# Vegeta2020/SE-SSD

Measured on NVIDIA H100. Metric: frames_per_sec, higher is better.
Workload: dtype f32

## Files before the change

### se-ssd_b200/csrc/bevconv_p2.cuh

```cuda
#pragma once
#include <cuda_fp16.h>

#include "tc_common.cuh"

namespace sessd {

constexpr int kP2TileU = 8, kP2TileV = 16;
constexpr int kP2MaxCopies = 6, kP2MaxRowsV = 18;
constexpr int kP2BStages = 6, kP2MaxBStages = 12;
constexpr int kP2MmaWarps = 8;
constexpr int kP2PatchWarp = 8, kP2WeightWarp = 9;
constexpr int kP2Threads = 320;
constexpr int kP2ThreadsRegA = 384, kP2RegsConsumer = 232, kP2RegsProducer = 40;
static_assert(2 * (kP2RegsConsumer - 168) <= 168 - kP2RegsProducer, "the consumers take what the producers release");
constexpr int kP2MaxSmem = 227 * 1024;
constexpr int kP2Chunk = 32;
constexpr int kP2ItemsHeader = 32;
enum { kP2Planes = 0, kP2SplitF16 = 1 };
enum { kP2NoProbe = 0, kP2ProbeClocks = 1, kP2ProbeLoads = 2 };

struct P2Params {
    int batch, cin, cout;
    int in_stride;
    int out_h, out_w;
// ... 27 lines not shown
    kProfItems,
    kProfSteps,
    kProfItemClk,
    kProfBFull,
    kProfPatchFull,
    kProfMmaWait,
    kProfEpilogue,
    kProfPatchEmpty,
    kProfPatchTotal,
    kProfBEmpty,
    kProfBTotal,
    kP2ProfWords = 16
};

__device__ __forceinline__ int p2_item_count(const P2Params &p) { return p.items ? __ldg(p.items) : p.total; }
__device__ __forceinline__ int p2_item(const P2Params &p, int k) { return p.items ? __ldg(p.items + kP2ItemsHeader + k) : k; }

struct P2ItemIndex { int rank, nb, t; };
__host__ __device__ __forceinline__ P2ItemIndex p2_item_index(int g, int nblocks, int tiles) {
    const int rank = g / (nblocks * tiles), rem = g - rank * (nblocks * tiles), nb = rem / tiles;
    return {rank, nb, rem - nb * tiles};
}

struct P2Item { int cls, n0, b, u0, v0, ntaps; };

__device__ __forceinline__ P2Item p2_decode(const P2Params &p, int g) {
    P2Item it;
    const P2ItemIndex ix = p2_item_index(g, p.nblocks, p.tiles);
    int t = ix.t;
    it.cls = p.cls_order[ix.rank];
    it.n0 = ix.nb * p.n_tile;
    const int tu = t % p.tiles_u; t /= p.tiles_u;
    const int tv = t % p.tiles_v;
    it.b = t / p.tiles_v;
    it.u0 = tu * kP2TileU; it.v0 = tv * kP2TileV;
    it.ntaps = p.cls_ntaps[it.cls];
    return it;
}

template <int N>
__device__ __forceinline__ void p2_wgmma(float *d, uint64_t da, uint64_t db, uint32_t accumulate) {
    if constexpr (N == 32) wgmma_f16_n32(d, da, db, accumulate);
    else if constexpr (N == 64) wgmma_f16_n64(d, da, db, accumulate);
    else if constexpr (N == 128) wgmma_f16_n128(d, da, db, accumulate);
    else wgmma_f16_n256(d, da, db, accumulate);
}

template <int N>
__device__ __forceinline__ void p2_wgmma_ra(float *d, const uint32_t *a, uint64_t db, uint32_t accumulate) {
    if constexpr (N == 32) wgmma_f16_ra_n32(d, a, db, accumulate);
    else if constexpr (N == 64) wgmma_f16_ra_n64(d, a, db, accumulate);
    else if constexpr (N == 128) wgmma_f16_ra_n128(d, a, db, accumulate);
    else wgmma_f16_ra_n256(d, a, db, accumulate);
}

__device__ __forceinline__ void p2_quad_transpose(const float *s, int q, float v[8]) {
    const bool odd = q & 1, up = q & 2;
    float a[2][2][2];
#pragma unroll
    for (int k = 0; k < 2; ++k)
#pragma unroll
        for (int e = 0; e < 2; ++e) {
            const float even_g = s[4 * (2 * k) + e], odd_g = s[4 * (2 * k + 1) + e];
            const float keep = odd ? odd_g : even_g;
            const float recv = __shfl_xor_sync(0xFFFFFFFFu, odd ? even_g : odd_g, 1);
            a[k][0][e] = odd ? recv : keep;
            a[k][1][e] = odd ? keep : recv;
        }
#pragma unroll
    for (int b = 0; b < 2; ++b)
#pragma unroll
        for (int e = 0; e < 2; ++e) {
            const float keep = up ? a[1][b][e] : a[0][b][e];
            const float recv = __shfl_xor_sync(0xFFFFFFFFu, up ? a[0][b][e] : a[1][b][e], 2);
            v[2 * b + e] = up ? recv : keep;
            v[2 * (2 + b) + e] = up ? keep : recv;
        }
}

template <bool PROFILE>
__device__ __forceinline__ long long p2_tick() {
    if constexpr (PROFILE) return clock64();
    return 0;
}
template <bool PROFILE>
__device__ __forceinline__ void p2_tock(long long &clk, long long t0) {
    if constexpr (PROFILE) clk += clock64() - t0;
}

__device__ __forceinline__ void p2_split_patch(const P2Params &p, const unsigned char *staging, unsigned char *planes, float s_in, int ctid) {
    const int rows = p.rows_v * kP2TileU;
    const int copy_in = p.staging_bytes / p.ncopies;
    const int items = p.ncopies * rows * 4;
    for (int i = ctid; i < items; i += kP2MmaWarps * 32) {
        const int j = i & 3, r = (i >> 2) % rows, c = (i >> 2) / rows;
        unsigned char *hi = planes + 2 * c * p.copy_bytes + r * 64 + ((j ^ ((r >> 1) & 3)) << 4);
        const float4 *src = reinterpret_cast<const float4 *>(staging + c * copy_in + r * 128 + j * 32);
        const float4 a = src[0], b = src[1];
        const float x[8] = {a.x * s_in, a.y * s_in, a.z * s_in, a.w * s_in, b.x * s_in, b.y * s_in, b.z * s_in, b.w * s_in};
        __align__(16) __half h[8], l[8];
#pragma unroll
        for (int t = 0; t < 8; ++t) { h[t] = __float2half_rn(x[t]); l[t] = __float2half_rn(x[t] - __half2float(h[t])); }
        *reinterpret_cast<uint4 *>(hi) = *reinterpret_cast<const uint4 *>(h);
        *reinterpret_cast<uint4 *>(hi + p.copy_bytes) = *reinterpret_cast<const uint4 *>(l);
    }
    asm volatile("fence.proxy.async.shared::cta;\n" ::: "memory");
    asm volatile("bar.sync 1, %0;\n" ::"n"(kP2MmaWarps * 32) : "memory");
}

template <int NT, int MODE, bool REGA = false, int PROBE = kP2NoProbe>
__global__ void __launch_bounds__(REGA ? kP2ThreadsRegA : kP2Threads, 1) bev_conv_p2_kernel(const __grid_constant__ CUtensorMap map_a,
                                                                   const __grid_constant__ CUtensorMap map_b,
                                                                   const float *__restrict__ scale, const float *__restrict__ shift,
                                                                   const float *__restrict__ resid, float *__restrict__ out_f32,
                                                                   __half *__restrict__ out_planes, P2Params p) {
    static_assert(!REGA || MODE == kP2Planes, "register-fed A reads the TMA-written planes");
    constexpr bool PROFILE = PROBE != kP2NoProbe, LOADS_ONLY = PROBE == kP2ProbeLoads;
    extern __shared__ unsigned char smem_raw[];
    unsigned char *tiles = (unsigned char *)(((uintptr_t)smem_raw + 1023) & ~(uintptr_t)1023);
    unsigned char *patches = tiles + p.bring_bytes;
    unsigned char *staging = patches + p.npatch * p.patch_bytes;
    uint64_t *bars = (uint64_t *)(staging + p.npatch * p.staging_bytes);
    uint64_t *patch_full = bars, *patch_empty = bars + 2, *b_full = bars + 4, *b_empty = bars + 4 + kP2MaxBStages;
    uint32_t *s_aoff = (uint32_t *)(b_empty + kP2MaxBStages);
    float *s_scale = (float *)(((uintptr_t)(s_aoff + 4 * 9) + 15) & ~(uintptr_t)15), *s_shift = s_scale + p.cout;

    const int warp = threadIdx.x >> 5, lane = threadIdx.x & 31;
    if (threadIdx.x == kP2PatchWarp * 32) prefetch_tensormap(&map_a);
    if (threadIdx.x == kP2WeightWarp * 32) prefetch_tensormap(&map_b);
    const int nchunks = p.cin / kP2Chunk;
// ... 197 lines not shown
                        first = false;
                        if constexpr (PROFILE) ++clk[kProfSteps];
                        { const long long t0 = p2_tick<PROFILE>(); wgmma_wait<1>(); p2_tock<PROFILE>(clk[kProfMmaWait], t0); }
                        if (lane == 0) {
                            if (prevS >= 0) mbar_arrive(&b_empty[prevS]);
                            if (prev_pb >= 0) mbar_arrive(&patch_empty[prev_pb]);
                        }
                        prevS = S;
                        prev_pb = (tap == ntaps - 1) ? pb : -1;
                        if (++S == p.bstages) { S = 0; bph ^= 1u; }
                    }
                    if (p.npatch == 1) {
                        { const long long t0 = p2_tick<PROFILE>(); wgmma_wait<0>(); p2_tock<PROFILE>(clk[kProfMmaWait], t0); }
                        if (lane == 0) {
                            mbar_arrive(&b_empty[prevS]);
                            mbar_arrive(&patch_empty[pb]);
                        }
                        prevS = prev_pb = -1;
                    }
                    if (++pb == p.npatch) { pb = 0; pph ^= 1u; }
                }
            }
            { const long long t0 = p2_tick<PROFILE>(); wgmma_wait<0>(); p2_tock<PROFILE>(clk[kProfMmaWait], t0); }
            const long long t_epi = p2_tick<PROFILE>();
            wgmma_fence_regs<NT>(acc);
            if (lane == 0) {
                if (prevS >= 0) mbar_arrive(&b_empty[prevS]);
                if (prev_pb >= 0) mbar_arrive(&patch_empty[prev_pb]);
            }
#pragma unroll
            for (int i = 0; i < kAcc; ++i) acc[i] = acc[kAcc + i] + acc[i];
            const P2Item it = p2_decode(p, g);
            const int q = lane & 3;
            const int r0 = wg * 64 + wq * 16 + (lane >> 2);
            bool rows_ok[2];
            size_t opixs[2];
#pragma unroll
            for (int h = 0; h < 2; ++h) {
                const int r = r0 + 8 * h;
                const int lv = r / kP2TileU, lu = r % kP2TileU;
                const int gu = it.u0 + lu, gv = it.v0 + lv;
                rows_ok[h] = it.b < p.batch && gu < p.grid_u && gv < p.grid_v;
                const int ou = gu * p.out_stride + p.cls_off_u[it.cls], ov = gv * p.out_stride + p.cls_off_v[it.cls];
                const int oy = p.u_is_x ? ov : ou, ox = p.u_is_x ? ou : ov;
                opixs[h] = ((size_t)it.b * p.out_h + (size_t)oy) * p.out_w + (size_t)ox;
            }
#pragma unroll
            for (int j = 0; j < (LOADS_ONLY ? 0 : NT / 32); ++j)
#pragma unroll
                for (int h = 0; h < 2; ++h) {
                    const bool row_ok = rows_ok[h];
                    const size_t opix = opixs[h];
                    float v[8], o[8] = {};
                    p2_quad_transpose(acc + 16 * j + 2 * h, q, v);
                    const int n = it.n0 + 32 * j + 8 * q;
                    const size_t off = opix * p.cout + n;
                    if (row_ok && n < p.cout) {
                        float sc[8], sh[8];
#pragma unroll
                        for (int t = 0; t < 8; t += 4) {
                            const float4 a = *reinterpret_cast<const float4 *>(s_scale + n + t);
                            const float4 b = *reinterpret_cast<const float4 *>(s_shift + n + t);
                            sc[t] = a.x; sc[t + 1] = a.y; sc[t + 2] = a.z; sc[t + 3] = a.w;
                            sh[t] = b.x; sh[t + 1] = b.y; sh[t + 2] = b.z; sh[t + 3] = b.w;
                        }
#pragma unroll
                        for (int t = 0; t < 8; ++t) {
                            o[t] = fmaf(v[t] * inv_sa, sc[t], sh[t]);
                            if (p.relu) o[t] = fmaxf(o[t], 0.f);
                        }
                        if (resid) {
#pragma unroll
                            for (int t = 0; t < 8; t += 4) {
                                const float4 rr = __ldg(reinterpret_cast<const float4 *>(resid + off + t));
                                o[t] += rr.x; o[t + 1] += rr.y; o[t + 2] += rr.z; o[t + 3] += rr.w;
                            }
                        }
#pragma unroll
                        for (int t = 0; t < 8; ++t) vmax = fmaxf(vmax, fabsf(o[t]));
                        if (out_planes) {
                            __align__(16) __half2 hi[4], lo[4];
#pragma unroll
                            for (int t = 0; t < 4; ++t) {
                                const float x0 = o[2 * t] * s_out, x1 = o[2 * t + 1] * s_out;
                                hi[t] = __floats2half2_rn(x0, x1);
                                const float2 f = __half22float2(hi[t]);
                                lo[t] = __floats2half2_rn(x0 - f.x, x1 - f.y);
                            }
                            *reinterpret_cast<uint4 *>(out_planes + off) = *reinterpret_cast<const uint4 *>(hi);
                            *reinterpret_cast<uint4 *>(out_planes + p.out_plane_stride + off) = *reinterpret_cast<const uint4 *>(lo);
                        }
                    }
                    if (out_f32) {
                        const bool up = q & 2;
                        float keep[4], recv[4];
#pragma unroll
                        for (int t = 0; t < 4; ++t) {
                            keep[t] = up ? o[4 + t] : o[t];
                            recv[t] = __shfl_xor_sync(0xFFFFFFFFu, up ? o[t] : o[4 + t], 2);
                        }
                        const int n_lo = it.n0 + 32 * j + 8 * (q & 1), c_lo = n_lo + 4 * (q >> 1);
                        const float4 w_lo = up ? make_float4(recv[0], recv[1], recv[2], recv[3]) : make_float4(keep[0], keep[1], keep[2], keep[3]);
                        const float4 w_hi = up ? make_float4(keep[0], keep[1], keep[2], keep[3]) : make_float4(recv[0], recv[1], recv[2], recv[3]);
                        if (row_ok && n_lo < p.cout) *reinterpret_cast<float4 *>(out_f32 + opix * p.cout + c_lo) = w_lo;
                        if (row_ok && n_lo + 16 < p.cout) *reinterpret_cast<float4 *>(out_f32 + opix * p.cout + c_lo + 16) = w_hi;
                    }
                }
// ... 274 lines not shown
```

### se-ssd_b200/csrc/spconv_cg.cu

```cuda
#include <cuda_fp16.h>

#include "tc_common.cuh"
#include "tile_lists.cuh"

namespace sessd {

constexpr int kCgBM = 128;
constexpr int kCgMaxK = 27;
constexpr int kCgProdWarps = 8;
constexpr int kCgMmaWarps = 8;
constexpr int kCgWeightWarp = kCgProdWarps + kCgMmaWarps;
constexpr int kCgThreads = (kCgWeightWarp + 1) * 32;

template <int CP, int COUT, int DEEP = 0>
struct CgCfg {
    static constexpr bool kWide = (CP == 64);
    static constexpr int kATile = (kWide ? 2 : 1) * kCgBM * 128;
    static constexpr int kBTile = (kWide ? 2 : 1) * COUT * 128;
    static constexpr int kStage = kATile + (kBTile + 1023) / 1024 * 1024;
    static constexpr int kStages = (kWide ? 2 : 4) * (DEEP ? 2 : 1);
    static constexpr int kMeta = kCgBM * kCgMaxK * 4  + kCgMaxK * 16  + 32 * 4  + 33 * 4  + 32 * 4  +
                                 3 * kStages * 8  + 24;
    static constexpr int kSmem = kStages * kStage + kMeta + 1024;
    static constexpr int kCPO = COUT > 32 ? 64 : 32;
};

struct CgArgs {
    const __half *planes;
    const float *in_info;
    const unsigned int *tiles;
    int tile_stride;
    const int *d_n_out;
    int kvol, max_out, relu;
    const float *scale, *shift;
    float gain, shift_max;
    float *out_f32;
    __half *out_planes;
    float *out_info;
};

__device__ __forceinline__ void cg_cp_async16(uint32_t smem_dst, const void *gsrc) {
    asm volatile("cp.async.cg.shared.global [%0], [%1], 16;\n" ::"r"(smem_dst), "l"(gsrc) : "memory");
}
__device__ __forceinline__ void cg_fence_proxy_async() { asm volatile("fence.proxy.async.shared::cta;\n" ::: "memory"); }
__device__ __forceinline__ void cg_sts_zero16(uint32_t saddr) {
    asm volatile("st.shared.v4.b32 [%0], {%1, %1, %1, %1};\n" ::"r"(saddr), "r"(0) : "memory");
}

template <int COUT>
__device__ __forceinline__ void cg_wgmma(float *d, uint64_t da, uint64_t db, uint32_t accumulate) {
    if constexpr (COUT == 32) wgmma_f16_n32(d, da, db, accumulate);
    else wgmma_f16_n64(d, da, db, accumulate);
}

template <int CP, int COUT, int DEEP>
__global__ void __launch_bounds__(kCgThreads, 1) spconv_cg_kernel(const __grid_constant__ CUtensorMap map_w, const CgArgs a) {
    using C = CgCfg<CP, COUT, DEEP>;
    const int n_out = min(*a.d_n_out, a.max_out);
    const int ntiles = (n_out + kCgBM - 1) / kCgBM;
    if ((int)blockIdx.x >= ntiles) return;
    const int kvol = a.kvol;
    if (threadIdx.x == kCgWeightWarp * 32) prefetch_tensormap(&map_w);

    extern __shared__ unsigned char smem_raw[];
    unsigned char *tiles = (unsigned char *)(((uintptr_t)smem_raw + 1023) & ~(uintptr_t)1023);
    uint32_t *s_list = (uint32_t *)(tiles + C::kStages * C::kStage);
    uint32_t *s_valid = s_list + kCgBM * kCgMaxK;
    int *s_cnt = (int *)(s_valid + kCgMaxK * 4);
    int *s_klist = s_cnt + 32;
    int *s_nact = s_klist + 32;
    int *s_off = s_nact + 1;
    uint64_t *bars = (uint64_t *)(((uintptr_t)(s_off + 32) + 7) & ~(uintptr_t)7);
    uint64_t *full_a = bars, *full_b = bars + C::kStages, *empty = bars + 2 * C::kStages;

    const int tid = threadIdx.x, warp = tid >> 5, lane = tid & 31;
    const uint32_t tiles_u32 = smem_u32(tiles);

    if (tid == 0) {
        for (int s = 0; s < C::kStages; ++s) { mbar_init(&full_a[s], kCgProdWarps / C::kStages); mbar_init(&full_b[s], 1); mbar_init(&empty[s], kCgMmaWarps); }
        asm volatile("fence.mbarrier_init.release.cluster;\n" ::: "memory");
    }
    for (int s = 0; s < C::kStages; ++s)
        for (int o = tid * 16; o < C::kATile; o += kCgThreads * 16) cg_sts_zero16(tiles_u32 + (uint32_t)(s * C::kStage + o));
    cg_fence_proxy_async();
    __syncthreads();

    const float amax_in = __ldg(a.in_info), s_in = __ldg(a.in_info + 1);
    const float inv_act = 1.f / s_in;
    const float s_out = pow2_scale_for_bound(amax_in * a.gain + a.shift_max);
    if (blockIdx.x == 0 && tid == 0 && a.out_info) a.out_info[1] = s_out;
    float vmax = 0.f;
    uint32_t dirty[4] = {0u, 0u, 0u, 0u};
    int st0 = 0;
    uint32_t ph0 = 0;

    for (int tile = blockIdx.x; tile < ntiles; tile += gridDim.x) {
        const int row0 = tile * kCgBM;
        const int rows = min(kCgBM, n_out - row0);
        {
            const unsigned int *rec = a.tiles + (size_t)tile * (size_t)a.tile_stride;
            const int c = (int)__ldg(rec + lane);
            unsigned int spec[4];
#pragma unroll
            for (int u = 0; u < 4; ++u) spec[u] = (tid + u * kCgThreads < kTlRows * kvol) ? __ldg(rec + kTlHeader + tid + u * kCgThreads) : 0u;
            const int incl = warp_incl_scan(c, lane);
            const int total = __shfl_sync(0xffffffffu, incl, 31);
            if (warp == 0) {
                s_cnt[lane] = c;
                s_off[lane] = incl - c;
                const unsigned int m = __ballot_sync(0xffffffffu, c > 0);
                if (c > 0) s_klist[__popc(m & ((1u << lane) - 1u))] = lane;
                if (lane == 0) *s_nact = __popc(m);
            }
            if (tid < kvol * 4) s_valid[tid] = __ldg(rec + kTlMask + tid);
#pragma unroll
            for (int u = 0; u < 4; ++u)
                if (tid + u * kCgThreads < total) s_list[tid + u * kCgThreads] = spec[u];
            for (int e = tid + 4 * kCgThreads; e < total; e += kCgThreads) s_list[e] = __ldg(rec + kTlHeader + e);
        }
        __syncthreads();
        const int nact = *s_nact;

        if (warp == kCgWeightWarp) {
            int s = st0;
            uint32_t ph = ph0;
            for (int j = 0; j < nact; ++j) {
                const int k = s_klist[j];
                mbar_wait(&empty[s], ph ^ 1u);
                if (elect_one()) {
                    mbar_expect_tx(&full_b[s], C::kBTile);
                    unsigned char *b_tile = tiles + s * C::kStage + C::kATile;
                    tma_load_4d(b_tile, &map_w, &full_b[s], 0, 0, 0, k);
                    tma_load_4d(b_tile + C::kBTile / 2, &map_w, &full_b[s], 0, 0, 1, k);
                }
                __syncwarp();
                if (++s == C::kStages) { s = 0; ph ^= 1u; }
            }
        } else if (warp >= kCgProdWarps) {
            const int cw = warp - kCgProdWarps, wg = cw >> 2, wq = cw & 3;
            constexpr int kAcc = COUT / 2;
            float acc_m[kAcc], acc_c[kAcc];
#pragma unroll
            for (int i = 0; i < kAcc; ++i) { acc_m[i] = 0.f; acc_c[i] = 0.f; }
            const uint32_t a_rows = (uint32_t)(wg * 64 * 128);
            int s = st0, prev = -1;
            uint32_t ph = ph0;
            for (int j = 0; j < nact; ++j) {
                mbar_wait(&full_b[s], ph);
                mbar_wait(&full_a[s], ph);
                const uint32_t st = tiles_u32 + (uint32_t)(s * C::kStage);
                const uint64_t dA = kDescSw128Hi | desc_lo(st + a_rows);
                const uint32_t first = j != 0 ? 1u : 0u;
                wgmma_fence();
                if constexpr (C::kWide) {
                    const uint64_t dAl = dA + ((kCgBM * 128) >> 4);
                    const uint64_t dBh = kDescSw128Hi | desc_lo(st + C::kATile);
                    const uint64_t dBl = dBh + ((COUT * 128) >> 4);
#pragma unroll
                    for (int kk = 0; kk < 4; ++kk) cg_wgmma<COUT>(acc_m, dA + 2 * kk, dBh + 2 * kk, first | (kk != 0));
#pragma unroll
                    for (int kk = 0; kk < 4; ++kk) cg_wgmma<COUT>(acc_c, dA + 2 * kk, dBl + 2 * kk, first | (kk != 0));
#pragma unroll
                    for (int kk = 0; kk < 4; ++kk) cg_wgmma<COUT>(acc_c, dAl + 2 * kk, dBh + 2 * kk, 1u);
                } else {
                    const uint64_t dBh = kDescSw64Hi | desc_lo(st + C::kATile);
                    const uint64_t dBl = dBh + ((COUT * 64) >> 4);
#pragma unroll
                    for (int kk = 0; kk < 2; ++kk) cg_wgmma<COUT>(acc_m, dA + 2 * kk, dBh + 2 * kk, first | (kk != 0));
#pragma unroll
                    for (int kk = 0; kk < 2; ++kk) cg_wgmma<COUT>(acc_c, dA + 2 * kk, dBl + 2 * kk, first | (kk != 0));
#pragma unroll
                    for (int kk = 0; kk < 2; ++kk) cg_wgmma<COUT>(acc_c, dA + 4 + 2 * kk, dBh + 2 * kk, 1u);
                }
                wgmma_commit();
                wgmma_wait<1>();
                if (prev >= 0 && lane == 0) mbar_arrive(&empty[prev]);
                prev = s;
                if (++s == C::kStages) { s = 0; ph ^= 1u; }
            }
            wgmma_wait<0>();
            wgmma_fence_regs<kAcc>(acc_m);
            wgmma_fence_regs<kAcc>(acc_c);
            if (prev >= 0 && lane == 0) mbar_arrive(&empty[prev]);
            const int r0 = wg * 64 + wq * 16 + (lane >> 2);
            const int c2 = 2 * (lane & 3);
#pragma unroll
            for (int h = 0; h < 2; ++h) {
                const int r = r0 + 8 * h;
                if (r >= rows) continue;
                const size_t orow = (size_t)(row0 + r);
#pragma unroll
                for (int g = 0; g < COUT / 8; ++g) {
                    const int n = 8 * g + c2, i = 4 * g + 2 * h;
                    const float2 sc = __ldg(reinterpret_cast<const float2 *>(a.scale + n));
                    const float2 sh = a.shift ? __ldg(reinterpret_cast<const float2 *>(a.shift + n)) : make_float2(0.f, 0.f);
                    float o0 = fmaf((acc_m[i] + acc_c[i]) * inv_act, sc.x, sh.x);
                    float o1 = fmaf((acc_m[i + 1] + acc_c[i + 1]) * inv_act, sc.y, sh.y);
                    if (a.relu) { o0 = fmaxf(o0, 0.f); o1 = fmaxf(o1, 0.f); }
                    vmax = fmaxf(vmax, fmaxf(fabsf(o0), fabsf(o1)));
                    if (a.out_f32) *reinterpret_cast<float2 *>(a.out_f32 + orow * COUT + n) = make_float2(o0, o1);
                    if (a.out_planes) {
                        const float x0 = o0 * s_out, x1 = o1 * s_out;
                        const __half2 hi = __floats2half2_rn(x0, x1);
                        const float2 f = __half22float2(hi);
                        const __half2 lo = __floats2half2_rn(x0 - f.x, x1 - f.y);
                        __half2 *dst = reinterpret_cast<__half2 *>(a.out_planes + orow * (2 * C::kCPO) + n);
                        dst[0] = hi;
                        dst[C::kCPO / 2] = lo;
                    }
                }
            }
        } else {
            constexpr int kGroupWarps = kCgProdWarps / C::kStages;
            constexpr int kGroupThreads = kGroupWarps * 32;
            constexpr int kOwnRows = kCgBM / kGroupWarps;
            constexpr int kOwnWords = kOwnRows / 32;
            constexpr int kLanesPerRow = C::kWide ? 16 : 8;
            constexpr int kRowsPerPass = kGroupThreads / kLanesPerRow;
            const int grp = warp / kGroupWarps, gw = warp % kGroupWarps;
            const int gtid = tid - grp * kGroupThreads;
            const int slot = gtid / kLanesPerRow;
            const int c = gtid % kLanesPerRow;
            const int half = c >> 3, cc = c & 7;
            const uint32_t a_base = tiles_u32 + (uint32_t)(grp * C::kStage);
            for (int j = (grp - st0 + C::kStages) % C::kStages; j < nact; j += C::kStages) {
                const uint32_t ph = ph0 ^ ((uint32_t)((st0 + j) / C::kStages) & 1u);
                const int k = s_klist[j];
                if (lane == 0) mbar_wait(&empty[grp], ph ^ 1u);
                __syncwarp();
#pragma unroll
                for (int w = 0; w < kOwnWords; ++w) {
                    const uint32_t vs = s_valid[k * 4 + gw * kOwnWords + w];
                    const uint32_t z = dirty[w] & ~vs;
                    dirty[w] = vs;
                    if (z) {
#pragma unroll
                        for (int q4 = 0; q4 < 8; ++q4) {
                            const int r32 = q4 * 4 + (lane >> 3);
                            if ((z >> r32) & 1u) {
                                const uint32_t dst = a_base + (uint32_t)((gw * kOwnRows + w * 32 + r32) * 128 + (lane & 7) * 16);
                                cg_sts_zero16(dst);
                                if constexpr (C::kWide) cg_sts_zero16(dst + kCgBM * 128);
                            }
                        }
                    }
                }
                const int n = s_cnt[k];
                const uint32_t *lst = s_list + s_off[k];
                auto copy_row = [&](uint32_t e) {
                    const uint32_t r = tl_tile_row(e);
                    const size_t src = (size_t)tl_in_row(e);
                    if constexpr (C::kWide)
                        cg_cp_async16(a_base + (uint32_t)half * (kCgBM * 128) + r * 128u + (((uint32_t)cc ^ (r & 7u)) << 4),
                                      a.planes + src * 128 + half * 64 + cc * 8);
                    else
                        cg_cp_async16(a_base + r * 128u + (((uint32_t)cc ^ (r & 7u)) << 4), a.planes + src * 64 + cc * 8);
                };
                int i = slot;
                for (; i + 3 * kRowsPerPass < n; i += 4 * kRowsPerPass) {
                    const uint32_t e0 = lst[i], e1 = lst[i + kRowsPerPass], e2 = lst[i + 2 * kRowsPerPass], e3 = lst[i + 3 * kRowsPerPass];
                    copy_row(e0); copy_row(e1); copy_row(e2); copy_row(e3);
                }
                for (; i < n; i += kRowsPerPass) copy_row(lst[i]);
                asm volatile("cp.async.wait_all;\n" ::: "memory");
// ... 20 lines not shown
template <int CP, int COUT, int DEEP>
static int launch_spconv_cg(const CgArgs &a, const void *w_h2, cudaStream_t st) {
    using C = CgCfg<CP, COUT, DEEP>;
    static bool attr_done = false;
    if (!attr_done) {
        cudaError_t e = cudaFuncSetAttribute(spconv_cg_kernel<CP, COUT, DEEP>, cudaFuncAttributeMaxDynamicSharedMemorySize, C::kSmem);
        if (e != cudaSuccess) return (int)e;
        attr_done = true;
    }
    CUtensorMap map_w;
    int rc;
    if (C::kWide) {
        const cuuint64_t dims[4] = {64, (cuuint64_t)COUT, 2, (cuuint64_t)a.kvol};
        const cuuint32_t box[4] = {64, (cuuint32_t)COUT, 1, 1};
        rc = encode_map_4d(&map_w, w_h2, dims, box, nullptr, CU_TENSOR_MAP_DATA_TYPE_FLOAT16, 2);
    } else {
        EncodeTiledFn enc = get_tensor_map_encoder();
        if (!enc) return SESSD_EINVAL;
        const cuuint64_t dims[4] = {32, (cuuint64_t)COUT, 2, (cuuint64_t)a.kvol};
        const cuuint64_t strides[3] = {64, (cuuint64_t)COUT * 64, (cuuint64_t)COUT * 128};
        const cuuint32_t box[4] = {32, (cuuint32_t)COUT, 1, 1};
        const cuuint32_t estr[4] = {1, 1, 1, 1};
        CUresult r = enc(&map_w, CU_TENSOR_MAP_DATA_TYPE_FLOAT16, 4, const_cast<void *>(w_h2), dims, strides, box, estr, CU_TENSOR_MAP_INTERLEAVE_NONE,
                         CU_TENSOR_MAP_SWIZZLE_64B, CU_TENSOR_MAP_L2_PROMOTION_L2_128B, CU_TENSOR_MAP_FLOAT_OOB_FILL_NONE);
        rc = r == CUDA_SUCCESS ? 0 : 700 + (int)r;
    }
    if (rc) return rc;
    static int num_sms = 0;
    if (!num_sms) {
        int dev = 0;
        SESSD_CUDA_TRY(cudaGetDevice(&dev));
        SESSD_CUDA_TRY(cudaDeviceGetAttribute(&num_sms, cudaDevAttrMultiProcessorCount, dev));
    }
    const int tiles = div_up(a.max_out, kCgBM);
    const int grid = tiles < num_sms ? tiles : num_sms;
    SESSD_LAUNCH((spconv_cg_kernel<CP, COUT, DEEP>), grid, kCgThreads, C::kSmem, st, map_w, a);
    return last_error();
}

}

using namespace sessd;

extern "C" void sessd_set_sp_cg_deep(int on) { sessd::g_cg_deep = on ? 1 : 0; }

extern "C" int sessd_spconv_forward_cg(const void *d_in_planes, int cp, int plane_rows, const float *d_in_info, const void *d_tiles, int kvol,
                                       const int *d_n_out, int max_out, const void *d_weight_h2, int cout, const float *d_scale,
                                       const float *d_shift, int relu, float gain, float shift_max, float *d_out_f32, void *d_out_planes,
                                       float *d_out_info, void *stream) {
    if (!d_in_planes || !d_in_info || !d_tiles || !d_n_out || !d_weight_h2 || !d_scale || (!d_out_f32 && !d_out_planes) || max_out < 1 ||
        kvol < 1 || kvol > kCgMaxK || plane_rows < 1 || plane_rows > (1 << 25))
        return SESSD_EINVAL;
    if (d_out_planes && !d_out_info) return SESSD_EINVAL;
    CgArgs a;
    a.planes = (const __half *)d_in_planes; a.in_info = d_in_info; a.tiles = (const unsigned int *)d_tiles; a.tile_stride = tile_list_stride(kvol); a.d_n_out = d_n_out; a.kvol = kvol; a.max_out = max_out;
    a.relu = relu; a.scale = d_scale; a.shift = d_shift; a.gain = gain; a.shift_max = shift_max; a.out_f32 = d_out_f32;
    a.out_planes = (__half *)d_out_planes; a.out_info = d_out_info;
    cudaStream_t st = (cudaStream_t)stream;
#define SESSD_CG_CASE(CPV, CO) \
    if (cp == CPV && cout == CO) return g_cg_deep ? launch_spconv_cg<CPV, CO, 1>(a, d_weight_h2, st) : launch_spconv_cg<CPV, CO, 0>(a, d_weight_h2, st);
    SESSD_CG_CASE(32, 32)
    SESSD_CG_CASE(32, 64)
    SESSD_CG_CASE(64, 32)
    SESSD_CG_CASE(64, 64)
#undef SESSD_CG_CASE
    return SESSD_EINVAL;
}
```

### se-ssd_b200/csrc/tc_common.cuh

```cuda
#pragma once
#include <cuda.h>

#include "common.cuh"

namespace sessd {

__device__ __forceinline__ uint32_t smem_u32(const void *p) { return (uint32_t)__cvta_generic_to_shared(p); }

__device__ __forceinline__ void mbar_init(uint64_t *bar, int count) {
    asm volatile("mbarrier.init.shared::cta.b64 [%0], %1;\n" ::"r"(smem_u32(bar)), "r"(count));
}
__device__ __forceinline__ void mbar_expect_tx(uint64_t *bar, uint32_t bytes) {
    asm volatile("mbarrier.arrive.expect_tx.shared::cta.b64 _, [%0], %1;\n" ::"r"(smem_u32(bar)), "r"(bytes) : "memory");
}
__device__ __forceinline__ void mbar_arrive(uint64_t *bar) {
    asm volatile("mbarrier.arrive.shared::cta.b64 _, [%0];\n" ::"r"(smem_u32(bar)) : "memory");
}
__device__ __forceinline__ bool mbar_try_wait(uint64_t *bar, uint32_t parity) {
    uint32_t ok;
    asm volatile(
        "{\n\t.reg .pred p;\n\t"
        "mbarrier.try_wait.parity.shared::cta.b64 p, [%1], %2;\n\t"
        "selp.b32 %0, 1, 0, p;\n\t}\n"
        : "=r"(ok)
// ... 11 lines not shown
        asm volatile("mov.u64 %0, %%globaltimer;" : "=l"(t1));
        if (t1 - t0 > 2000000000ull) __trap();
    }
}
static __device__ __noinline__ void mbar_wait_slow(uint64_t *bar, uint32_t parity) { mbar_wait_spin(bar, parity); }
template <bool INLINE = false>
__device__ __forceinline__ void mbar_wait(uint64_t *bar, uint32_t parity) {
    if (mbar_try_wait(bar, parity)) return;
    if constexpr (INLINE) mbar_wait_spin(bar, parity);
    else mbar_wait_slow(bar, parity);
}

__device__ __forceinline__ void tma_load_4d(void *smem_dst, const CUtensorMap *map, uint64_t *bar, int c0, int c1, int c2, int c3) {
    asm volatile(
        "cp.async.bulk.tensor.4d.shared::cluster.global.mbarrier::complete_tx::bytes [%0], [%1, {%3, %4, %5, %6}], [%2];\n" ::"r"(
            smem_u32(smem_dst)),
        "l"(map), "r"(smem_u32(bar)), "r"(c0), "r"(c1), "r"(c2), "r"(c3)
        : "memory");
}
__device__ __forceinline__ void tma_load_5d(uint32_t smem_dst, const CUtensorMap *map, uint64_t *bar, int c0, int c1, int c2, int c3, int c4) {
    asm volatile(
        "cp.async.bulk.tensor.5d.shared::cluster.global.mbarrier::complete_tx::bytes [%0], [%1, {%3, %4, %5, %6, %7}], [%2];\n" ::"r"(smem_dst),
        "l"(map), "r"(smem_u32(bar)), "r"(c0), "r"(c1), "r"(c2), "r"(c3), "r"(c4)
        : "memory");
}

__device__ __forceinline__ void prefetch_tensormap(const CUtensorMap *m) {
    asm volatile("prefetch.tensormap [%0];\n" ::"l"(reinterpret_cast<uint64_t>(m)) : "memory");
}

__device__ __forceinline__ bool elect_one() {
    uint32_t pred;
    asm volatile("{\n\t.reg .pred p;\n\telect.sync _|p, 0xffffffff;\n\tselp.b32 %0, 1, 0, p;\n\t}\n" : "=r"(pred));
    return pred != 0;
}

__device__ __forceinline__ void ldsm_x4(uint32_t *r, uint32_t addr) {
    asm volatile("ldmatrix.sync.aligned.m8n8.x4.shared.b16 {%0,%1,%2,%3}, [%4];\n" : "=r"(r[0]), "=r"(r[1]), "=r"(r[2]), "=r"(r[3]) : "r"(addr) : "memory");
}

template <int N>
__device__ __forceinline__ void setmaxnreg_inc() { asm volatile("setmaxnreg.inc.sync.aligned.u32 %0;\n" ::"n"(N)); }
template <int N>
__device__ __forceinline__ void setmaxnreg_dec() { asm volatile("setmaxnreg.dec.sync.aligned.u32 %0;\n" ::"n"(N)); }

__device__ __forceinline__ void wgmma_fence() { asm volatile("wgmma.fence.sync.aligned;\n" ::: "memory"); }
__device__ __forceinline__ void wgmma_commit() { asm volatile("wgmma.commit_group.sync.aligned;\n" ::: "memory"); }
template <int N>
__device__ __forceinline__ void wgmma_wait() { asm volatile("wgmma.wait_group.sync.aligned %0;\n" ::"n"(N) : "memory"); }
template <int N>
__device__ __forceinline__ void wgmma_fence_regs(float *d) {
#pragma unroll
    for (int i = 0; i < N; ++i) asm volatile("" : "+f"(d[i])::"memory");
}

constexpr uint64_t kDescSw128Hi = ((uint64_t)(1024u >> 4) << 32) | ((uint64_t)1 << 62);
constexpr uint64_t kDescSw64Hi = ((uint64_t)(512u >> 4) << 32) | ((uint64_t)2 << 62);
__device__ __forceinline__ uint32_t desc_lo(uint32_t smem_addr) { return ((smem_addr >> 4) & 0x3FFFu) | (1u << 16); }

__device__ __forceinline__ void wgmma_f16_n32(float *d, uint64_t da, uint64_t db, uint32_t accumulate) {
    asm volatile(
        "{\n\t.reg .pred p;\n\t"
        "setp.ne.b32 p, %18, 0;\n\t"
        "wgmma.mma_async.sync.aligned.m64n32k16.f32.f16.f16 "
        "{%0, %1, %2, %3, %4, %5, %6, %7, %8, %9, %10, %11, %12, %13, %14, %15}, %16, %17, p, 1, 1, 0, 0;\n\t}\n"
        : "+f"(d[0]), "+f"(d[1]), "+f"(d[2]), "+f"(d[3]), "+f"(d[4]), "+f"(d[5]), "+f"(d[6]), "+f"(d[7]), "+f"(d[8]), "+f"(d[9]), "+f"(d[10]), "+f"(d[11]), "+f"(d[12]), "+f"(d[13]), "+f"(d[14]), "+f"(d[15])
        : "l"(da), "l"(db), "r"(accumulate));
}

__device__ __forceinline__ void wgmma_f16_n64(float *d, uint64_t da, uint64_t db, uint32_t accumulate) {
    asm volatile(
        "{\n\t.reg .pred p;\n\t"
        "setp.ne.b32 p, %34, 0;\n\t"
        "wgmma.mma_async.sync.aligned.m64n64k16.f32.f16.f16 "
        "{%0, %1, %2, %3, %4, %5, %6, %7, %8, %9, %10, %11, %12, %13, %14, %15, %16, %17, %18, %19, %20, %21, %22, %23, %24, %25, %26, %27, %28, %29, %30, %31}, %32, %33, p, 1, 1, 0, 0;\n\t}\n"
        : "+f"(d[0]), "+f"(d[1]), "+f"(d[2]), "+f"(d[3]), "+f"(d[4]), "+f"(d[5]), "+f"(d[6]), "+f"(d[7]), "+f"(d[8]), "+f"(d[9]), "+f"(d[10]), "+f"(d[11]), "+f"(d[12]), "+f"(d[13]), "+f"(d[14]), "+f"(d[15]), "+f"(d[16]), "+f"(d[17]), "+f"(d[18]), "+f"(d[19]), "+f"(d[20]), "+f"(d[21]), "+f"(d[22]), "+f"(d[23]), "+f"(d[24]), "+f"(d[25]), "+f"(d[26]), "+f"(d[27]), "+f"(d[28]), "+f"(d[29]), "+f"(d[30]), "+f"(d[31])
        : "l"(da), "l"(db), "r"(accumulate));
}

__device__ __forceinline__ void wgmma_f16_n128(float *d, uint64_t da, uint64_t db, uint32_t accumulate) {
    asm volatile(
        "{\n\t.reg .pred p;\n\t"
        "setp.ne.b32 p, %66, 0;\n\t"
        "wgmma.mma_async.sync.aligned.m64n128k16.f32.f16.f16 "
        "{%0, %1, %2, %3, %4, %5, %6, %7, %8, %9, %10, %11, %12, %13, %14, %15, %16, %17, %18, %19, %20, %21, %22, %23, %24, %25, %26, %27, %28, %29, %30, %31, %32, %33, %34, %35, %36, %37, %38, %39, %40, %41, %42, %43, %44, %45, %46, %47, %48, %49, %50, %51, %52, %53, %54, %55, %56, %57, %58, %59, %60, %61, %62, %63}, %64, %65, p, 1, 1, 0, 0;\n\t}\n"
        : "+f"(d[0]), "+f"(d[1]), "+f"(d[2]), "+f"(d[3]), "+f"(d[4]), "+f"(d[5]), "+f"(d[6]), "+f"(d[7]), "+f"(d[8]), "+f"(d[9]), "+f"(d[10]), "+f"(d[11]), "+f"(d[12]), "+f"(d[13]), "+f"(d[14]), "+f"(d[15]), "+f"(d[16]), "+f"(d[17]), "+f"(d[18]), "+f"(d[19]), "+f"(d[20]), "+f"(d[21]), "+f"(d[22]), "+f"(d[23]), "+f"(d[24]), "+f"(d[25]), "+f"(d[26]), "+f"(d[27]), "+f"(d[28]), "+f"(d[29]), "+f"(d[30]), "+f"(d[31]), "+f"(d[32]), "+f"(d[33]), "+f"(d[34]), "+f"(d[35]), "+f"(d[36]), "+f"(d[37]), "+f"(d[38]), "+f"(d[39]), "+f"(d[40]), "+f"(d[41]), "+f"(d[42]), "+f"(d[43]), "+f"(d[44]), "+f"(d[45]), "+f"(d[46]), "+f"(d[47]), "+f"(d[48]), "+f"(d[49]), "+f"(d[50]), "+f"(d[51]), "+f"(d[52]), "+f"(d[53]), "+f"(d[54]), "+f"(d[55]), "+f"(d[56]), "+f"(d[57]), "+f"(d[58]), "+f"(d[59]), "+f"(d[60]), "+f"(d[61]), "+f"(d[62]), "+f"(d[63])
        : "l"(da), "l"(db), "r"(accumulate));
}

__device__ __forceinline__ void wgmma_f16_n256(float *d, uint64_t da, uint64_t db, uint32_t accumulate) {
    asm volatile(
        "{\n\t.reg .pred p;\n\t"
        "setp.ne.b32 p, %130, 0;\n\t"
        "wgmma.mma_async.sync.aligned.m64n256k16.f32.f16.f16 "
        "{%0, %1, %2, %3, %4, %5, %6, %7, %8, %9, %10, %11, %12, %13, %14, %15, %16, %17, %18, %19, %20, %21, %22, %23, %24, %25, %26, %27, %28, %29, %30, %31, %32, %33, %34, %35, %36, %37, %38, %39, %40, %41, %42, %43, %44, %45, %46, %47, %48, %49, %50, %51, %52, %53, %54, %55, %56, %57, %58, %59, %60, %61, %62, %63, %64, %65, %66, %67, %68, %69, %70, %71, %72, %73, %74, %75, %76, %77, %78, %79, %80, %81, %82, %83, %84, %85, %86, %87, %88, %89, %90, %91, %92, %93, %94, %95, %96, %97, %98, %99, %100, %101, %102, %103, %104, %105, %106, %107, %108, %109, %110, %111, %112, %113, %114, %115, %116, %117, %118, %119, %120, %121, %122, %123, %124, %125, %126, %127}, %128, %129, p, 1, 1, 0, 0;\n\t}\n"
        : "+f"(d[0]), "+f"(d[1]), "+f"(d[2]), "+f"(d[3]), "+f"(d[4]), "+f"(d[5]), "+f"(d[6]), "+f"(d[7]), "+f"(d[8]), "+f"(d[9]), "+f"(d[10]), "+f"(d[11]), "+f"(d[12]), "+f"(d[13]), "+f"(d[14]), "+f"(d[15]), "+f"(d[16]), "+f"(d[17]), "+f"(d[18]), "+f"(d[19]), "+f"(d[20]), "+f"(d[21]), "+f"(d[22]), "+f"(d[23]), "+f"(d[24]), "+f"(d[25]), "+f"(d[26]), "+f"(d[27]), "+f"(d[28]), "+f"(d[29]), "+f"(d[30]), "+f"(d[31]), "+f"(d[32]), "+f"(d[33]), "+f"(d[34]), "+f"(d[35]), "+f"(d[36]), "+f"(d[37]), "+f"(d[38]), "+f"(d[39]), "+f"(d[40]), "+f"(d[41]), "+f"(d[42]), "+f"(d[43]), "+f"(d[44]), "+f"(d[45]), "+f"(d[46]), "+f"(d[47]), "+f"(d[48]), "+f"(d[49]), "+f"(d[50]), "+f"(d[51]), "+f"(d[52]), "+f"(d[53]), "+f"(d[54]), "+f"(d[55]), "+f"(d[56]), "+f"(d[57]), "+f"(d[58]), "+f"(d[59]), "+f"(d[60]), "+f"(d[61]), "+f"(d[62]), "+f"(d[63]), "+f"(d[64]), "+f"(d[65]), "+f"(d[66]), "+f"(d[67]), "+f"(d[68]), "+f"(d[69]), "+f"(d[70]), "+f"(d[71]), "+f"(d[72]), "+f"(d[73]), "+f"(d[74]), "+f"(d[75]), "+f"(d[76]), "+f"(d[77]), "+f"(d[78]), "+f"(d[79]), "+f"(d[80]), "+f"(d[81]), "+f"(d[82]), "+f"(d[83]), "+f"(d[84]), "+f"(d[85]), "+f"(d[86]), "+f"(d[87]), "+f"(d[88]), "+f"(d[89]), "+f"(d[90]), "+f"(d[91]), "+f"(d[92]), "+f"(d[93]), "+f"(d[94]), "+f"(d[95]), "+f"(d[96]), "+f"(d[97]), "+f"(d[98]), "+f"(d[99]), "+f"(d[100]), "+f"(d[101]), "+f"(d[102]), "+f"(d[103]), "+f"(d[104]), "+f"(d[105]), "+f"(d[106]), "+f"(d[107]), "+f"(d[108]), "+f"(d[109]), "+f"(d[110]), "+f"(d[111]), "+f"(d[112]), "+f"(d[113]), "+f"(d[114]), "+f"(d[115]), "+f"(d[116]), "+f"(d[117]), "+f"(d[118]), "+f"(d[119]), "+f"(d[120]), "+f"(d[121]), "+f"(d[122]), "+f"(d[123]), "+f"(d[124]), "+f"(d[125]), "+f"(d[126]), "+f"(d[127])
        : "l"(da), "l"(db), "r"(accumulate));
}

__device__ __forceinline__ void wgmma_f16_ra_n32(float *d, const uint32_t *a, uint64_t db, uint32_t accumulate) {
    asm volatile(
        "{\n\t.reg .pred p;\n\t"
        "setp.ne.b32 p, %21, 0;\n\t"
        "wgmma.mma_async.sync.aligned.m64n32k16.f32.f16.f16 "
        "{%0, %1, %2, %3, %4, %5, %6, %7, %8, %9, %10, %11, %12, %13, %14, %15}, {%16, %17, %18, %19}, %20, p, 1, 1, 0;\n\t}\n"
        : "+f"(d[0]), "+f"(d[1]), "+f"(d[2]), "+f"(d[3]), "+f"(d[4]), "+f"(d[5]), "+f"(d[6]), "+f"(d[7]), "+f"(d[8]), "+f"(d[9]), "+f"(d[10]), "+f"(d[11]), "+f"(d[12]), "+f"(d[13]), "+f"(d[14]), "+f"(d[15])
// ... 63 lines not shown
```

Measured before the change: 1398.

## Merge split-fp16 wgmmas into one wide-N accumulator and vectorize spconv epilogue

The sparse conv consumer now issues a single wgmma with N=2*COUT covering both weight halves into one accumulator, then adds the halves at the end, instead of three separate N=COUT wgmmas into two accumulators. The TMA weight-load order is swapped so the low-plane weights sit first and can be read as one contiguous wide B tile. The epilogue caches scale and shift in shared memory, uses a quad transpose so each thread writes 16-byte vector stores for the half planes and the f32 output, and gains an alignment check. The wgmma wait changes from overlapping one group to waiting for completion on every step, which loses some overlap between MMA groups and the release of pipeline stages.

```diff
diff --git a/se-ssd_b200/csrc/bevconv_p2.cuh b/se-ssd_b200/csrc/bevconv_p2.cuh
--- a/se-ssd_b200/csrc/bevconv_p2.cuh
+++ b/se-ssd_b200/csrc/bevconv_p2.cuh
@@ -103,30 +103,6 @@
     else if constexpr (N == 64) wgmma_f16_ra_n64(d, a, db, accumulate);
     else if constexpr (N == 128) wgmma_f16_ra_n128(d, a, db, accumulate);
     else wgmma_f16_ra_n256(d, a, db, accumulate);
-}
-
-__device__ __forceinline__ void p2_quad_transpose(const float *s, int q, float v[8]) {
-    const bool odd = q & 1, up = q & 2;
-    float a[2][2][2];
-#pragma unroll
-    for (int k = 0; k < 2; ++k)
-#pragma unroll
-        for (int e = 0; e < 2; ++e) {
-            const float even_g = s[4 * (2 * k) + e], odd_g = s[4 * (2 * k + 1) + e];
-            const float keep = odd ? odd_g : even_g;
-            const float recv = __shfl_xor_sync(0xFFFFFFFFu, odd ? even_g : odd_g, 1);
-            a[k][0][e] = odd ? recv : keep;
-            a[k][1][e] = odd ? keep : recv;
-        }
-#pragma unroll
-    for (int b = 0; b < 2; ++b)
-#pragma unroll
-        for (int e = 0; e < 2; ++e) {
-            const float keep = up ? a[1][b][e] : a[0][b][e];
-            const float recv = __shfl_xor_sync(0xFFFFFFFFu, up ? a[0][b][e] : a[1][b][e], 2);
-            v[2 * b + e] = up ? recv : keep;
-            v[2 * (2 + b) + e] = up ? keep : recv;
-        }
 }
 
 template <bool PROFILE>
@@ -430,7 +406,7 @@
                     const bool row_ok = rows_ok[h];
                     const size_t opix = opixs[h];
                     float v[8], o[8] = {};
-                    p2_quad_transpose(acc + 16 * j + 2 * h, q, v);
+                    quad_transpose8(acc + 16 * j + 2 * h, q, v);
                     const int n = it.n0 + 32 * j + 8 * q;
                     const size_t off = opix * p.cout + n;
                     if (row_ok && n < p.cout) {
diff --git a/se-ssd_b200/csrc/spconv_cg.cu b/se-ssd_b200/csrc/spconv_cg.cu
--- a/se-ssd_b200/csrc/spconv_cg.cu
+++ b/se-ssd_b200/csrc/spconv_cg.cu
@@ -19,8 +19,8 @@
     static constexpr int kBTile = (kWide ? 2 : 1) * COUT * 128;
     static constexpr int kStage = kATile + (kBTile + 1023) / 1024 * 1024;
     static constexpr int kStages = (kWide ? 2 : 4) * (DEEP ? 2 : 1);
-    static constexpr int kMeta = kCgBM * kCgMaxK * 4  + kCgMaxK * 16  + 32 * 4  + 33 * 4  + 32 * 4  +
-                                 3 * kStages * 8  + 24;
+    static constexpr int kMeta = kCgBM * kCgMaxK * 4  + kCgMaxK * 16  + 2 * COUT * 4  + 32 * 4  +
+                                 33 * 4  + 32 * 4  + 3 * kStages * 8  + 24;
     static constexpr int kSmem = kStages * kStage + kMeta + 1024;
     static constexpr int kCPO = COUT > 32 ? 64 : 32;
 };
@@ -47,10 +47,11 @@
     asm volatile("st.shared.v4.b32 [%0], {%1, %1, %1, %1};\n" ::"r"(saddr), "r"(0) : "memory");
 }
 
-template <int COUT>
+template <int N>
 __device__ __forceinline__ void cg_wgmma(float *d, uint64_t da, uint64_t db, uint32_t accumulate) {
-    if constexpr (COUT == 32) wgmma_f16_n32(d, da, db, accumulate);
-    else wgmma_f16_n64(d, da, db, accumulate);
+    if constexpr (N == 32) wgmma_f16_n32(d, da, db, accumulate);
+    else if constexpr (N == 64) wgmma_f16_n64(d, da, db, accumulate);
+    else wgmma_f16_n128(d, da, db, accumulate);
 }
 
 template <int CP, int COUT, int DEEP>
@@ -66,7 +67,9 @@
     unsigned char *tiles = (unsigned char *)(((uintptr_t)smem_raw + 1023) & ~(uintptr_t)1023);
     uint32_t *s_list = (uint32_t *)(tiles + C::kStages * C::kStage);
     uint32_t *s_valid = s_list + kCgBM * kCgMaxK;
-    int *s_cnt = (int *)(s_valid + kCgMaxK * 4);
+    float *s_scale = (float *)(s_valid + kCgMaxK * 4);
+    float *s_shift = s_scale + COUT;
+    int *s_cnt = (int *)(s_shift + COUT);
     int *s_klist = s_cnt + 32;
     int *s_nact = s_klist + 32;
     int *s_off = s_nact + 1;
@@ -79,6 +82,10 @@
     if (tid == 0) {
         for (int s = 0; s < C::kStages; ++s) { mbar_init(&full_a[s], kCgProdWarps / C::kStages); mbar_init(&full_b[s], 1); mbar_init(&empty[s], kCgMmaWarps); }
         asm volatile("fence.mbarrier_init.release.cluster;\n" ::: "memory");
+    }
+    if (tid < COUT) {
+        s_scale[tid] = __ldg(a.scale + tid);
+        s_shift[tid] = a.shift ? __ldg(a.shift + tid) : 0.f;
     }
     for (int s = 0; s < C::kStages; ++s)
         for (int o = tid * 16; o < C::kATile; o += kCgThreads * 16) cg_sts_zero16(tiles_u32 + (uint32_t)(s * C::kStage + o));
@@ -130,8 +137,8 @@
                 if (elect_one()) {
                     mbar_expect_tx(&full_b[s], C::kBTile);
                     unsigned char *b_tile = tiles + s * C::kStage + C::kATile;
-                    tma_load_4d(b_tile, &map_w, &full_b[s], 0, 0, 0, k);
-                    tma_load_4d(b_tile + C::kBTile / 2, &map_w, &full_b[s], 0, 0, 1, k);
+                    tma_load_4d(b_tile + C::kBTile / 2, &map_w, &full_b[s], 0, 0, 0, k);
+                    tma_load_4d(b_tile, &map_w, &full_b[s], 0, 0, 1, k);
                 }
                 __syncwarp();
                 if (++s == C::kStages) { s = 0; ph ^= 1u; }
@@ -139,11 +146,11 @@
         } else if (warp >= kCgProdWarps) {
             const int cw = warp - kCgProdWarps, wg = cw >> 2, wq = cw & 3;
             constexpr int kAcc = COUT / 2;
-            float acc_m[kAcc], acc_c[kAcc];
-#pragma unroll
-            for (int i = 0; i < kAcc; ++i) { acc_m[i] = 0.f; acc_c[i] = 0.f; }
+            float acc[COUT];
+#pragma unroll
+            for (int i = 0; i < COUT; ++i) acc[i] = 0.f;
             const uint32_t a_rows = (uint32_t)(wg * 64 * 128);
-            int s = st0, prev = -1;
+            int s = st0;
             uint32_t ph = ph0;
             for (int j = 0; j < nact; ++j) {
                 mbar_wait(&full_b[s], ph);
@@ -154,62 +161,87 @@
                 wgmma_fence();
                 if constexpr (C::kWide) {
                     const uint64_t dAl = dA + ((kCgBM * 128) >> 4);
-                    const uint64_t dBh = kDescSw128Hi | desc_lo(st + C::kATile);
-                    const uint64_t dBl = dBh + ((COUT * 128) >> 4);
-#pragma unroll
-                    for (int kk = 0; kk < 4; ++kk) cg_wgmma<COUT>(acc_m, dA + 2 * kk, dBh + 2 * kk, first | (kk != 0));
-#pragma unroll
-                    for (int kk = 0; kk < 4; ++kk) cg_wgmma<COUT>(acc_c, dA + 2 * kk, dBl + 2 * kk, first | (kk != 0));
-#pragma unroll
-                    for (int kk = 0; kk < 4; ++kk) cg_wgmma<COUT>(acc_c, dAl + 2 * kk, dBh + 2 * kk, 1u);
+                    const uint64_t dBl = kDescSw128Hi | desc_lo(st + C::kATile);
+                    const uint64_t dBh = dBl + ((COUT * 128) >> 4);
+#pragma unroll
+                    for (int kk = 0; kk < 4; ++kk) cg_wgmma<2 * COUT>(acc, dA + 2 * kk, dBl + 2 * kk, first | (kk != 0));
+#pragma unroll
+                    for (int kk = 0; kk < 4; ++kk) cg_wgmma<COUT>(acc, dAl + 2 * kk, dBh + 2 * kk, 1u);
                 } else {
-                    const uint64_t dBh = kDescSw64Hi | desc_lo(st + C::kATile);
-                    const uint64_t dBl = dBh + ((COUT * 64) >> 4);
-#pragma unroll
-                    for (int kk = 0; kk < 2; ++kk) cg_wgmma<COUT>(acc_m, dA + 2 * kk, dBh + 2 * kk, first | (kk != 0));
-#pragma unroll
-                    for (int kk = 0; kk < 2; ++kk) cg_wgmma<COUT>(acc_c, dA + 2 * kk, dBl + 2 * kk, first | (kk != 0));
-#pragma unroll
-                    for (int kk = 0; kk < 2; ++kk) cg_wgmma<COUT>(acc_c, dA + 4 + 2 * kk, dBh + 2 * kk, 1u);
+                    const uint64_t dBl = kDescSw64Hi | desc_lo(st + C::kATile);
+                    const uint64_t dBh = dBl + ((COUT * 64) >> 4);
+#pragma unroll
+                    for (int kk = 0; kk < 2; ++kk) cg_wgmma<2 * COUT>(acc, dA + 2 * kk, dBl + 2 * kk, first | (kk != 0));
+#pragma unroll
+                    for (int kk = 0; kk < 2; ++kk) cg_wgmma<COUT>(acc, dA + 4 + 2 * kk, dBh + 2 * kk, 1u);
                 }
                 wgmma_commit();
-                wgmma_wait<1>();
-                if (prev >= 0 && lane == 0) mbar_arrive(&empty[prev]);
-                prev = s;
+                wgmma_wait<0>();
+                if (lane == 0) mbar_arrive(&empty[s]);
                 if (++s == C::kStages) { s = 0; ph ^= 1u; }
             }
-            wgmma_wait<0>();
-            wgmma_fence_regs<kAcc>(acc_m);
-            wgmma_fence_regs<kAcc>(acc_c);
-            if (prev >= 0 && lane == 0) mbar_arrive(&empty[prev]);
+            wgmma_fence_regs<COUT>(acc);
+#pragma unroll
+            for (int i = 0; i < kAcc; ++i) acc[i] = acc[kAcc + i] + acc[i];
+            const int q = lane & 3;
             const int r0 = wg * 64 + wq * 16 + (lane >> 2);
-            const int c2 = 2 * (lane & 3);
-#pragma unroll
-            for (int h = 0; h < 2; ++h) {
-                const int r = r0 + 8 * h;
-                if (r >= rows) continue;
-                const size_t orow = (size_t)(row0 + r);
-#pragma unroll
-                for (int g = 0; g < COUT / 8; ++g) {
-                    const int n = 8 * g + c2, i = 4 * g + 2 * h;
-                    const float2 sc = __ldg(reinterpret_cast<const float2 *>(a.scale + n));
-                    const float2 sh = a.shift ? __ldg(reinterpret_cast<const float2 *>(a.shift + n)) : make_float2(0.f, 0.f);
-                    float o0 = fmaf((acc_m[i] + acc_c[i]) * inv_act, sc.x, sh.x);
-                    float o1 = fmaf((acc_m[i + 1] + acc_c[i + 1]) * inv_act, sc.y, sh.y);
-                    if (a.relu) { o0 = fmaxf(o0, 0.f); o1 = fmaxf(o1, 0.f); }
-                    vmax = fmaxf(vmax, fmaxf(fabsf(o0), fabsf(o1)));
-                    if (a.out_f32) *reinterpret_cast<float2 *>(a.out_f32 + orow * COUT + n) = make_float2(o0, o1);
-                    if (a.out_planes) {
-                        const float x0 = o0 * s_out, x1 = o1 * s_out;
-                        const __half2 hi = __floats2half2_rn(x0, x1);
-                        const float2 f = __half22float2(hi);
-                        const __half2 lo = __floats2half2_rn(x0 - f.x, x1 - f.y);
-                        __half2 *dst = reinterpret_cast<__half2 *>(a.out_planes + orow * (2 * C::kCPO) + n);
-                        dst[0] = hi;
-                        dst[C::kCPO / 2] = lo;
-                    }
-                }
-            }
+#pragma unroll
+            for (int jb = 0; jb < COUT / 32; ++jb)
+#pragma unroll
+                for (int h = 0; h < 2; ++h) {
+                    const int r = r0 + 8 * h;
+                    const bool row_ok = r < rows;
+                    const size_t orow = (size_t)(row0 + r);
+                    float v[8], o[8];
+                    quad_transpose8(acc + 16 * jb + 2 * h, q, v);
+                    const int n = 32 * jb + 8 * q;
+#pragma unroll
+                    for (int t = 0; t < 8; t += 4) {
+                        const float4 sc = *reinterpret_cast<const float4 *>(s_scale + n + t);
+                        const float4 sh = *reinterpret_cast<const float4 *>(s_shift + n + t);
+                        o[t] = fmaf(v[t] * inv_act, sc.x, sh.x);
+                        o[t + 1] = fmaf(v[t + 1] * inv_act, sc.y, sh.y);
+                        o[t + 2] = fmaf(v[t + 2] * inv_act, sc.z, sh.z);
+                        o[t + 3] = fmaf(v[t + 3] * inv_act, sc.w, sh.w);
+                    }
+                    if (a.relu) {
+#pragma unroll
+                        for (int t = 0; t < 8; ++t) o[t] = fmaxf(o[t], 0.f);
+                    }
+                    if (row_ok) {
+#pragma unroll
+                        for (int t = 0; t < 8; ++t) vmax = fmaxf(vmax, fabsf(o[t]));
+                    }
+                    if (a.out_planes && row_ok) {
+                        __align__(16) __half2 hi[4], lo[4];
+#pragma unroll
+                        for (int t = 0; t < 4; ++t) {
+                            const float x0 = o[2 * t] * s_out, x1 = o[2 * t + 1] * s_out;
+                            hi[t] = __floats2half2_rn(x0, x1);
+                            const float2 f = __half22float2(hi[t]);
+                            lo[t] = __floats2half2_rn(x0 - f.x, x1 - f.y);
+                        }
+                        __half *dst = a.out_planes + orow * (2 * C::kCPO) + n;
+                        *reinterpret_cast<uint4 *>(dst) = *reinterpret_cast<const uint4 *>(hi);
+                        *reinterpret_cast<uint4 *>(dst + C::kCPO) = *reinterpret_cast<const uint4 *>(lo);
+                    }
+                    if (a.out_f32) {
+                        const bool up = q & 2;
+                        float keep[4], recv[4];
+#pragma unroll
+                        for (int t = 0; t < 4; ++t) {
+                            keep[t] = up ? o[4 + t] : o[t];
+                            recv[t] = __shfl_xor_sync(0xFFFFFFFFu, up ? o[t] : o[4 + t], 2);
+                        }
+                        const float4 w_lo = up ? make_float4(recv[0], recv[1], recv[2], recv[3]) : make_float4(keep[0], keep[1], keep[2], keep[3]);
+                        const float4 w_hi = up ? make_float4(keep[0], keep[1], keep[2], keep[3]) : make_float4(recv[0], recv[1], recv[2], recv[3]);
+                        float *dst = a.out_f32 + orow * COUT + 32 * jb + 8 * (q & 1) + 4 * (q >> 1);
+                        if (row_ok) {
+                            *reinterpret_cast<float4 *>(dst) = w_lo;
+                            *reinterpret_cast<float4 *>(dst + 16) = w_hi;
+                        }
+                    }
+                }
         } else {
             constexpr int kGroupWarps = kCgProdWarps / C::kStages;
             constexpr int kGroupThreads = kGroupWarps * 32;
@@ -336,6 +368,7 @@
         kvol < 1 || kvol > kCgMaxK || plane_rows < 1 || plane_rows > (1 << 25))
         return SESSD_EINVAL;
     if (d_out_planes && !d_out_info) return SESSD_EINVAL;
+    if (((uintptr_t)d_out_f32 | (uintptr_t)d_out_planes) & 15) return SESSD_EINVAL;
     CgArgs a;
     a.planes = (const __half *)d_in_planes; a.in_info = d_in_info; a.tiles = (const unsigned int *)d_tiles; a.tile_stride = tile_list_stride(kvol); a.d_n_out = d_n_out; a.kvol = kvol; a.max_out = max_out;
     a.relu = relu; a.scale = d_scale; a.shift = d_shift; a.gain = gain; a.shift_max = shift_max; a.out_f32 = d_out_f32;
diff --git a/se-ssd_b200/csrc/tc_common.cuh b/se-ssd_b200/csrc/tc_common.cuh
--- a/se-ssd_b200/csrc/tc_common.cuh
+++ b/se-ssd_b200/csrc/tc_common.cuh
@@ -87,6 +87,30 @@
 __device__ __forceinline__ void wgmma_fence_regs(float *d) {
 #pragma unroll
     for (int i = 0; i < N; ++i) asm volatile("" : "+f"(d[i])::"memory");
+}
+
+__device__ __forceinline__ void quad_transpose8(const float *s, int q, float v[8]) {
+    const bool odd = q & 1, up = q & 2;
+    float a[2][2][2];
+#pragma unroll
+    for (int k = 0; k < 2; ++k)
+#pragma unroll
+        for (int e = 0; e < 2; ++e) {
+            const float even_g = s[4 * (2 * k) + e], odd_g = s[4 * (2 * k + 1) + e];
+            const float keep = odd ? odd_g : even_g;
+            const float recv = __shfl_xor_sync(0xFFFFFFFFu, odd ? even_g : odd_g, 1);
+            a[k][0][e] = odd ? recv : keep;
+            a[k][1][e] = odd ? keep : recv;
+        }
+#pragma unroll
+    for (int b = 0; b < 2; ++b)
+#pragma unroll
+        for (int e = 0; e < 2; ++e) {
+            const float keep = up ? a[1][b][e] : a[0][b][e];
+            const float recv = __shfl_xor_sync(0xFFFFFFFFu, up ? a[0][b][e] : a[1][b][e], 2);
+            v[2 * b + e] = up ? recv : keep;
+            v[2 * (2 + b) + e] = up ? keep : recv;
+        }
 }
 
 constexpr uint64_t kDescSw128Hi = ((uint64_t)(1024u >> 4) << 32) | ((uint64_t)1 << 62);
```

Measured after the change: 1465, median of 6. 4.8% higher.
